# alex-petrenko/megaverse

Measured on NVIDIA H100. Metric: agent obs/sec (whole box), higher is better.
Workload: dtype f32

## Files before the change

### megaverse_b200/capi.py

```python
import ctypes as C
import os

import numpy as np

_PKG = os.path.dirname(os.path.abspath(__file__))
LIB_PATH = os.environ.get("MV_B200_LIB") or os.path.join(_PKG, "libmegaverse_b200.so")
_lib = None

MV_OK, MV_ERR_ARG, MV_ERR_CUDA, MV_ERR_CAPACITY, MV_ERR_STATE = 0, -1, -2, -3, -4
MV_END_NONE, MV_END_TIME, MV_END_SOLVED, MV_END_REQUESTED = 0, 1, 2, 3
MV_SEG_NONE, MV_SEG_STATIC, MV_SEG_TERRAIN, MV_SEG_OBJECT, MV_SEG_AGENT, MV_SEG_REWARD = 0, 1, 2, 3, 4, 5


class MegaverseError(RuntimeError):
    def __init__(self, code, msg):
        super().__init__("megaverse_b200 error %d: %s" % (code, msg))
        self.code = code


def lib():
    global _lib
    if _lib is None:
        if not os.path.exists(LIB_PATH):
            raise ImportError("%s is missing: run `python -m megaverse_b200._build` (needs nvcc)" % LIB_PATH)
# ... 382 lines not shown

    def static_cap(self):
        lib().mv_debug_static_cap.argtypes = [C.c_void_p]
        return int(lib().mv_debug_static_cap(self._h))

    def raster_config(self):
        out = (C.c_int32 * 4)()
        lib().mv_debug_raster_config.argtypes = [C.c_void_p, C.c_void_p]
        self._ck(lib().mv_debug_raster_config(self._h, out))
        return {"grid": out[0], "ctas_per_sm": out[1], "smem": out[2], "bands": out[3]}

    def raster_stats(self, enable=True, read=True):
        out = (C.c_ulonglong * 16)()
        lib().mv_debug_raster_stats.argtypes = [C.c_void_p, C.c_void_p, C.c_int]
        self._ck(lib().mv_debug_raster_stats(self._h, out if read else None, 1 if enable else 0))
        names = ["work_items", "instances", "visible_instances", "items", "clipped_items", "triangles", "batches", "sub_passes", "cyc_head", "cyc_tma_wait", "cyc_instance", "cyc_item", "cyc_tile", "cyc_total"]
        return {n: int(out[i]) for i, n in enumerate(names)}

    def states_create(self, rows):
        sid = C.c_int()
        self._ck(lib().mv_states_create(self._h, int(rows), C.byref(sid)))
        return sid.value

    def states_save(self, store, envs, rows):
        e, r = np.ascontiguousarray(envs, dtype=np.int32), np.ascontiguousarray(rows, dtype=np.int32)
        assert e.size == r.size
        self._ck(lib().mv_states_save(self._h, int(store), e.ctypes.data, r.ctypes.data, e.size))

    def states_load(self, store, rows, envs):
        r, e = np.ascontiguousarray(rows, dtype=np.int32), np.ascontiguousarray(envs, dtype=np.int32)
        assert e.size == r.size
# ... 130 lines not shown
```

### megaverse_b200/csrc/engine.cu

```cuda
#include <cuda_runtime.h>

#include <algorithm>
#include <atomic>
#include <cctype>
#include <cmath>
#include <condition_variable>
#include <cstddef>
#include <cstdio>
#include <cstring>
#include <deque>
#include <functional>
#include <map>
#include <memory>
#include <mutex>
#include <optional>
#include <queue>
#include <string>
#include <thread>
#include <vector>

#include "../../include/megaverse_b200.h"
#include "hostmath.hpp"
#include "level_set.h"
#include "levelgen.hpp"
// ... 111 lines not shown
        std::vector<MvLevel> level;
        std::vector<std::vector<MvBox>> statics;
        std::vector<std::vector<float>> staticRot;
        std::vector<std::vector<MvDeco>> deco;
        std::vector<std::vector<uint32_t>> solid;
    };
    std::vector<HostRow> host;
    void free() { for (auto &s : slabs) s.free(); for (auto &s : stateSlabs) s.free(); }
};

}

static void fillConsts(MvConsts &k, int W, int H);
static_assert(MV_STATE_OBJECT_ROWS == MV_MAX_OBJECTS && MV_STATE_REWARD_ROWS == MV_MAX_REWARD, "state tensor rows");

static mvr::ViewParams frameParams(int W, int H, int bands, int bandRows, unsigned long long *spill, int triCap, const MvConsts &k) {
    mvr::ViewParams vp = {};
    vp.W = W; vp.H = H; vp.bands = bands; vp.bandRows = bandRows; vp.spill = spill; vp.spillStride = W * bandRows; vp.triCap = triCap;
    vp.p00 = k.p00; vp.p11 = k.p11; vp.p22 = k.p22; vp.p32 = k.p32;
    return vp;
}

constexpr int kMaxRasterWidth = 768;

static int hiresBandRows(int w) { return std::max(1, 96 / (w / 32)) * 4; }
static bool hiresSizeOk(int w, int hgt) { return w >= 32 && hgt >= 4 && w % 32 == 0 && hgt % 4 == 0 && w <= kMaxRasterWidth && hgt <= 4096; }
template <typename B> static cudaError_t ensureCapacity(B &b, size_t count) {
    if (b.p && b.n >= count) return cudaSuccess;
    b.free();
    return b.alloc(count);
}

using ViewKernel = void (*)(mvr::ViewParams);
// ... 15 lines not shown
}

struct mv_engine {
    std::string error;
    void setError(const std::string &e) { error = e; }

    int W = 0, H = 0, E = 0, A = 0, N = 0, threads = 1, device = 0;
    std::vector<std::string> envScenarioName;
    std::vector<int> envScenario;
    std::vector<std::vector<std::pair<std::string, float>>> shaping;
    std::vector<mv::LevelGenerator> gens;
    std::mt19937 master{std::random_device{}()};
    std::unique_ptr<WorkerPool> pool;

    int gridCells = 0, gridWords = 0;
    int triCap = 368;
    std::atomic<int> maxObjSeen{0};
    bool wantDepth = false, obsToHost = true, didReset = false, fastShading = true;
    bool wantSeg = false;
    bool hostStepPending = false;
    bool skipUnfitLevels = false;
    std::atomic<int> levelsSkipped{0};
    int zeroCopyOpt = 1, hostSlicesOpt = 0;
    bool rasterToHost = false;
    bool deliverToHost = false;
    bool deviceObsFresh = false;
    bool hostObsFresh = false, ownDeviceObsFresh = false;
    bool ownDeviceBuffers() const { return obsOut == d_obs.p && (!wantDepth || depthOut == d_depth.p); }
    int sliceCount = 1;
    cudaStream_t copyStream = nullptr;
    std::vector<cudaEvent_t> sliceEv;
// ... 35 lines not shown
    DevBuf<int32_t> d_actions;
    DevBuf<float> d_rtable;
    DevBuf<float> d_rewards;
    DevBuf<uint8_t> d_dones;
    DevBuf<uint8_t> d_doneReasons;
    DevBuf<float> d_trueObj;
    DevBuf<uint8_t> d_obs;
    DevBuf<float> d_depth;
    DevBuf<uint16_t> d_seg;
    uint8_t *obsOut = nullptr;
    float *depthOut = nullptr;
    DevBuf<int32_t> d_faults;
    DevBuf<uint32_t> d_workCounter;
    uint32_t counterBase = 0;
    DevBuf<unsigned long long> d_spill;
    DevBuf<unsigned long long> d_rasterStats;
    DevBuf<uint32_t> d_viewCost;
    size_t costItems() const { return size_t(N) * size_t(H / 4); }
    int rasterGridCap = 0;
    int rasterSched = 1;
    int rasterGrid = 0, rasterCtasPerSM = 0, rasterBands = 1, bandRows = 0;
    size_t rasterSmem = 0;
    struct Hires {
        int W = 0, H = 0;
        DevBuf<uint8_t> d_obs; PinBuf<uint8_t> h_obs;
        DevBuf<unsigned long long> spill;
        void free() { d_obs.free(); h_obs.free(); spill.free(); W = H = 0; }
    } hires;
    struct Cameras {
        DevBuf<int32_t> d_env; DevBuf<float> d_views;
// ... 359 lines not shown
            if (timed) MV_CUDA(cudaEventRecord(evRays, stream));
            if (const int rc = castRays(false, sp.active)) return rc;
            if (final) { if (const int rc = castRays(true, nullptr)) return rc; }
        }
        if (const int rc = endTimes(dep ? Timed::Union : Timed::Split, timed, final, nRays > 0)) return rc;
        return (nRays && !async) ? downloadRays(stream) : MV_OK;
    }
    int endTimes(Timed kind, bool timed = true, bool hadFinal = false, bool hadRays = false) {
        if (timed) MV_CUDA(cudaEventRecord(ev[2], stream));
        timedAs = kind;
        lastHadFinal = timed && hadFinal;
        lastHadRays = timed && hadRays;
        return MV_OK;
    }
    int launchFinal(bool toHost) {
        mvr::ViewParams vp = frameParams(W, H, rasterBands, bandRows, d_spill.p, triCap, consts);
        vp.instances = d_termInst.p; vp.instCounts = d_termCounts.p; vp.views = d_termViews.p;
        vp.obs = toHost ? h_finalObs.p : d_finalObs.p; vp.depth = wantDepth ? (toHost ? h_finalDepth.p : d_finalDepth.p) : nullptr;
        vp.viewBase = 0; vp.N = N;
        vp.envMask = d_dones.p;
        finalOnDevice = !toHost;
        return launchView(vp, false, mvr::Items::Ended);
    }
    int rasterGridFor(const mvr::ViewParams &vp) const {
        const int full = vp.camEnv ? cameraGrid : (vp.envMask ? maskedGrid : rasterGrid);
        return std::min(rasterGridCap > 0 ? std::min(full, rasterGridCap) : full, vp.N * vp.bands);
    }
    int launchView(mvr::ViewParams &vp, bool dependent, mvr::Items items = mvr::Items::All) {
        const int grid = rasterGridFor(vp);
        vp.A = A; vp.instStride = instCap;
        vp.workCounter = d_workCounter.p; vp.counterBase = counterBase;
// ... 2 lines not shown
        cfg.gridDim = dim3(unsigned(grid)); cfg.blockDim = dim3(mvr::kThreads); cfg.dynamicSmemBytes = rasterSmem; cfg.stream = stream;
        cudaLaunchAttribute attr[1];
        attr[0].id = cudaLaunchAttributeProgrammaticStreamSerialization;
        attr[0].val.programmaticStreamSerializationAllowed = 1;
        cfg.attrs = attr; cfg.numAttrs = dependent ? 1 : 0;
        MV_CUDA(cudaLaunchKernelEx(&cfg, viewKernelOf(items, vp.seg != nullptr, fastShading), vp));
        launches += 1;
        return MV_OK;
    }
    cudaError_t resetViewOrder() {
        std::vector<uint32_t> init(costItems() + size_t(E) + 1, 0u);
        for (int e = 0; e < E; ++e) init[costItems() + size_t(e)] = uint32_t(e);
        return cudaMemcpy(d_viewCost.p, init.data(), sizeof(uint32_t) * init.size(), cudaMemcpyHostToDevice);
    }
    int launchRaster(bool dep, const uint8_t *active) {
        mvr::ViewParams vp = frameParams(W, H, rasterBands, bandRows, d_spill.p, triCap, consts);
        vp.instances = d_inst.p; vp.instCounts = d_instCounts.p; vp.views = d_views.p;
        vp.obs = rasterToHost ? h_obs.p : obsOut; vp.depth = wantDepth ? (rasterToHost ? h_depth.p : depthOut) : nullptr;
        vp.seg = wantSeg ? (rasterToHost ? h_seg.p : d_seg.p) : nullptr;
        vp.stats = d_rasterStats.p;
        vp.ready = dep ? d_ready.p : nullptr; vp.readyStamp = dep ? readyStamp : 0;
        const bool fresh = rasterToHost ? hostObsFresh : (ownDeviceObsFresh && ownDeviceBuffers());
        const uint8_t *mask = fresh ? active : nullptr;
        const mvr::Items items = mask ? mvr::Items::Active : mvr::Items::All;
        vp.envMask = mask;
        deviceObsFresh = !rasterToHost;
        ownDeviceObsFresh = !rasterToHost && ownDeviceBuffers();
        hostObsFresh = deliverToHost;
        if (sliceCount <= 1) {
            vp.viewBase = 0; vp.N = N;
            if (rasterSched == 2 || (rasterSched == 1 && N * rasterBands > rasterGridFor(vp))) {
// ... 56 lines not shown
        vp.instances = d_inst.p; vp.instCounts = d_instCounts.p; vp.views = d_views.p;
        vp.obs = hires.d_obs.p;
        vp.viewBase = 0; vp.N = N;
        rc = launchView(vp, false);
        if (rc) return rc;
        MV_CUDA(cudaMemcpyAsync(hires.h_obs.p, hires.d_obs.p, size_t(N) * w * hgt * 4, cudaMemcpyDeviceToHost, stream));
        MV_CUDA(cudaStreamSynchronize(stream));
        return MV_OK;
    }
    int bandedFrame(int w, int hgt, int grid, DevBuf<unsigned long long> &spill, mvr::ViewParams &vp) {
        const int rowsPerBand = hiresBandRows(w);
        const int bands = (hgt + rowsPerBand - 1) / rowsPerBand;
        if (ensureCapacity(spill, size_t(grid) * w * rowsPerBand) != cudaSuccess) { setError("raster spill slab allocation failed"); return MV_ERR_CUDA; }
        MvConsts k;
        fillConsts(k, w, hgt);
        vp = frameParams(w, hgt, bands, rowsPerBand, spill.p, triCap, k);
        return MV_OK;
    }
    int launchCameras(const int32_t *dEnv, const float *dViews, int n, int w, int hgt, uint8_t *obs, float *depth, uint16_t *seg) {
        if (ensureCapacity(cams.d_range, 1) != cudaSuccess) { setError("camera counter allocation failed"); return MV_ERR_CUDA; }
        MV_CUDA(cudaMemsetAsync(cams.d_range.p, 0, sizeof(uint32_t), stream));
        if (n == 0) return MV_OK;
        mvr::ViewParams vp;
        const int rc = bandedFrame(w, hgt, cameraGrid, cams.spill, vp);
        if (rc) return rc;
        vp.instances = d_inst.p; vp.instCounts = d_instCounts.p; vp.views = dViews;
        vp.obs = obs; vp.depth = depth; vp.seg = seg;
        vp.viewBase = 0; vp.N = n;
        vp.camEnv = dEnv; vp.numEnvs = E; vp.rangeCount = cams.d_range.p;
        return launchView(vp, false, mvr::Items::Cameras);
    }
// ... 84 lines not shown
            maskedPerSM = v ? std::min(maskedPerSM, perSM) : perSM;
        }
        maskedGrid = numSMs * std::max(1, std::min(maskedPerSM, rasterCtasPerSM));
        int cameraPerSM = 0;
        for (int v = 0; v < 4; ++v) {
            const void *fn = reinterpret_cast<const void *>(viewKernelOf(mvr::Items::Cameras, v >= 2, v & 1));
            MV_CUDA(cudaFuncSetAttribute(fn, cudaFuncAttributeMaxDynamicSharedMemorySize, maxOptin));
            int perSM = 0;
            MV_CUDA(cudaOccupancyMaxActiveBlocksPerMultiprocessor(&perSM, fn, mvr::kThreads, rasterSmem));
            cameraPerSM = v ? std::min(cameraPerSM, perSM) : perSM;
        }
        cameraGrid = numSMs * std::max(1, std::min(cameraPerSM, rasterCtasPerSM));
        bandRows = ((H / 4 + rasterBands - 1) / rasterBands) * 4;
        d_spill.free();
        if (d_spill.alloc(size_t(rasterGrid) * W * bandRows) != cudaSuccess) { setError("raster spill slab allocation failed"); return MV_ERR_CUDA; }
        hires.free();
        return MV_OK;
    }

    void afterFlip(const uint8_t *flipped) {
        const int D = levelSlots;
        for (int e = 0; e < E; ++e) {
            if (!flipped || flipped[e]) {
                if (levelSet) { hostEpisode[size_t(e)] += 1; continue; }
                hostSlot[size_t(e)] = (hostSlot[size_t(e)] + 1) % D;
                hostEpisode[size_t(e)] += 1;
                scheduleGen(e, (hostSlot[size_t(e)] + D - 1) % D, hostEpisode[size_t(e)] + D - 1);
            }
        }
    }
// ... 347 lines not shown
        const int rc = quiesce();
        if (rc) return rc;
        MV_CUDA(cudaMemcpyAsync(&d_agents.p[size_t(env) * A + agent], w16, sizeof(float) * 16, cudaMemcpyHostToDevice, stream));
        MV_CUDA(cudaStreamSynchronize(stream));
        return MV_OK;
    }

    void freeAll() {
        if (pool) { pool->waitAll(); pool.reset(); }
        for (auto &st : stores) if (st) st->free();
        stores.clear();
        d_bankBase.free(); d_levelIds.free(); d_nextLevels.free(); h_levelIds.free(); h_nextLevels.free();
        h_pairs.free(); d_pairs.free(); h_envList.free(); d_envList.free(); h_active.free(); d_active.free();
        d_levels.free(); d_statics.free(); d_staticRot.free(); h_statics.free(); h_staticRot.free(); d_solid.free(); d_objGrid.free(); d_envs.free(); d_agents.free(); d_objects.free(); d_inst.free(); d_instCounts.free();
        d_views.free(); d_actions.free(); d_rtable.free(); d_rewards.free(); d_dones.free(); d_trueObj.free(); d_obs.free(); d_depth.free(); d_seg.free(); d_faults.free();
        hires.free(); cams.free(); d_deco.free(); h_deco.free(); d_prof.free(); d_ready.free(); d_workCounter.free(); d_spill.free(); d_rasterStats.free(); d_viewCost.free();
        h_levels.free(); h_solid.free(); h_actions.free(); h_rtable.free(); h_rewards.free(); h_dones.free(); h_trueObj.free(); h_obs.free(); h_depth.free(); h_seg.free();
        h_faults.free(); h_faultWord.free();
        d_doneReasons.free(); h_doneReasons.free();
        d_termInst.free(); d_termCounts.free(); d_termViews.free(); d_finalObs.free(); d_finalDepth.free(); h_finalObs.free(); h_finalDepth.free();
        d_state.free(); h_state.free();
        if (evState) { cudaEventDestroy(evState); evState = nullptr; }
        d_rayDirs.free(); d_rayDist.free(); d_rayTag.free(); h_rayDist.free(); h_rayTag.free();
        if (evRays) { cudaEventDestroy(evRays); evRays = nullptr; }
        for (auto &e : ev) if (e) { cudaEventDestroy(e); e = nullptr; }
        if (evFinal) { cudaEventDestroy(evFinal); evFinal = nullptr; }
        for (auto &p : ring) { if (p.ev) { cudaEventDestroy(p.ev); p.ev = nullptr; } p.rewards.free(); p.trueObj.free(); p.dones.free(); p.reasons.free(); p.levelIds.free(); }
        for (auto &e2 : sliceEv) if (e2) cudaEventDestroy(e2);
        sliceEv.clear();
        if (copyStream) { cudaStreamDestroy(copyStream); copyStream = nullptr; }
        if (stream) { cudaStreamDestroy(stream); stream = nullptr; }
// ... 1138 lines not shown
    int32_t cnt[8] = {0, n, 0, 0, 0, 0, 0, 0};
    for (int i = 0, last = 0; i < n; ++i) {
        MvInstance &d = inst[size_t(i)];
        d.mesh = int(inst18[i * 18]); d.color = int(inst18[i * 18 + 1]);
        std::memcpy(d.model, inst18 + i * 18 + 2, 64);
        d.pad[0] = i + 1; d.pad[1] = 0;
        if (d.mesh < last || d.mesh > 4 || d.color < 0 || d.color >= 22) return MV_ERR_ARG;
        last = d.mesh;
        cnt[d.mesh == 0 ? 0 : 1 + d.mesh] += 1;
    }
    MvConsts k;
    fillConsts(k, w, h);
    if (uploadPalette(&tmp) != MV_OK) return MV_ERR_CUDA;
    const ViewKernel fn = viewKernelOf(mvr::Items::All, wantSeg, fast);
    MvInstance *dInst = nullptr; int32_t *dCnt = nullptr; float *dView = nullptr, *dDepth = nullptr; uint8_t *dObs = nullptr; uint16_t *dSeg = nullptr;
    uint32_t *dCtr = nullptr; unsigned long long *dSpill = nullptr, *dStats = nullptr;
    const size_t px = size_t(w) * size_t(h);
    bool ok = cudaMalloc(&dInst, sizeof(MvInstance) * inst.size()) == cudaSuccess && cudaMalloc(&dCnt, 32) == cudaSuccess &&
              cudaMalloc(&dView, 64) == cudaSuccess && cudaMalloc(&dObs, px * 4) == cudaSuccess && cudaMalloc(&dDepth, px * 4) == cudaSuccess &&
              cudaMalloc(&dSeg, px * 2) == cudaSuccess && cudaMalloc(&dStats, 16 * sizeof(unsigned long long)) == cudaSuccess &&
              cudaMalloc(&dCtr, 16) == cudaSuccess && cudaMalloc(&dSpill, sizeof(unsigned long long) * size_t(bands) * size_t(w) * bandRows) == cudaSuccess &&
              cudaFuncSetAttribute(reinterpret_cast<const void *>(fn), cudaFuncAttributeMaxDynamicSharedMemorySize, maxOptin) == cudaSuccess;
    if (ok) {
        cudaMemcpy(dInst, inst.data(), sizeof(MvInstance) * inst.size(), cudaMemcpyHostToDevice);
        cudaMemcpy(dCnt, cnt, 32, cudaMemcpyHostToDevice);
        cudaMemcpy(dView, view16, 64, cudaMemcpyHostToDevice);
        cudaMemset(dCtr, 0, 16);
        cudaMemset(dStats, 0, 16 * sizeof(unsigned long long));
        mvr::ViewParams vp = frameParams(w, h, bands, bandRows, dSpill, triCap, k);
        vp.instances = dInst; vp.instCounts = dCnt; vp.views = dView; vp.instStride = int(inst.size()); vp.obs = dObs; vp.depth = depth ? dDepth : nullptr;
        vp.seg = wantSeg ? dSeg : nullptr; vp.stats = stats ? dStats : nullptr;
        vp.workCounter = dCtr; vp.viewBase = 0; vp.N = 1; vp.A = 1;
        fn<<<bands, mvr::kThreads, smem>>>(vp);
        ok = cudaDeviceSynchronize() == cudaSuccess;
        if (ok) {
            cudaMemcpy(rgba, dObs, px * 4, cudaMemcpyDeviceToHost);
            if (depth) cudaMemcpy(depth, dDepth, px * 4, cudaMemcpyDeviceToHost);
            if (wantSeg) cudaMemcpy(seg, dSeg, px * 2, cudaMemcpyDeviceToHost);
            if (stats) cudaMemcpy(stats, dStats, 16 * sizeof(unsigned long long), cudaMemcpyDeviceToHost);
        }
    }
    cudaFree(dCtr); cudaFree(dSpill); cudaFree(dInst); cudaFree(dCnt); cudaFree(dView); cudaFree(dObs); cudaFree(dDepth); cudaFree(dSeg); cudaFree(dStats);
    return ok ? MV_OK : MV_ERR_CUDA;
}

int mv_debug_render_instances(const float *view16, const float *inst18, int n, int w, int h, uint8_t *rgba, float *depth) {
    if (w < 32 || h < 4 || w % 32 || h % 4 || (w / 32) * (h / 4) > 128) return MV_ERR_ARG;
    const int opts[4] = {0, 0, 96, (h / 4) % 2 == 0 ? 2 : 1};
    return mv_debug_render_instances_ex(view16, inst18, n, w, h, opts, rgba, depth, nullptr, nullptr);
}

int mv_debug_cast_rays(const float *views16, const float *inst18, const int32_t *tags, const int32_t *counts, int E, int A, int stride,
                       const float *dirs3, int R, float max_dist, const uint8_t *env_mask, float *dist, uint16_t *tag) {
    if (!views16 || !inst18 || !tags || !counts || !dirs3 || !dist || !tag) return MV_ERR_ARG;
    if (E < 1 || E > 65536 || A < 1 || A > MV_MAX_AGENTS || R < 1 || R > MV_MAX_RAYS || stride < 1 || stride > 65536) return MV_ERR_ARG;
    if (size_t(E) * size_t(stride) > (size_t(1) << 22) || !std::isfinite(max_dist) || !(max_dist > 0.0f)) return MV_ERR_ARG;
    std::vector<MvInstance> inst(size_t(E) * size_t(stride));
// ... 70 lines not shown
```

### megaverse_b200/csrc/raster_view.cuh

```cuda
#pragma once
#include "dev_math.cuh"
#include "mesh_tables.inc"
#include "mv_types.h"

namespace mvr {
using namespace dm;

struct __align__(16) TriCover {
    long long C[3];
    int32_t A[3], B[3];
    float z[3];
    float invArea;
    uint32_t key;
    int32_t flags;
    uint32_t bx, by;
};
struct __align__(16) TriShade {
    float rw[3];
    float p[9];
    float n[9];
    float diffuse[3];
};
static_assert(sizeof(TriCover) == 80 && sizeof(TriShade) == 96, "triangle record layout");

// ... 44 lines not shown
    unsigned long long *stats;
    uint32_t *viewCost;
    uint32_t *order;
    uint32_t *exitCounter;
    unsigned long long *spill;
    int spillStride;
    int viewBase, N;
    int A, W, H;
    int bands, bandRows;
    int triCap;
    float p00, p11, p22, p32;
    const uint8_t *envMask;
    const int32_t *camEnv;
    uint32_t *rangeCount;
    int numEnvs;
};

struct SmemLayout { uint32_t stage, cover, shade, xf, off, frag, small, meshV, meshI, clip, slow, sched, misc, total; };
struct ViewMisc {
    float view[16];
    int32_t counts[8];
    int32_t nTris;
    int32_t nValid;
    int32_t tileCtr;
    uint32_t claim;
    int32_t prefetched;
    int32_t lastCta;
    int32_t wsum[kWarps];
    int32_t nSlow[2];
    uint32_t stat[8];
    alignas(8) unsigned long long bar[2];
    unsigned long long itemStart;
};
__host__ __device__ inline SmemLayout smemLayout(int triCap) {
    SmemLayout L;
    uint32_t o = 0;
    L.stage = o; o += 2u * kInstChunk * uint32_t(sizeof(MvInstance));
    L.cover = o; o += uint32_t(triCap) * uint32_t(sizeof(TriCover));
    L.shade = o; o += uint32_t(triCap) * uint32_t(sizeof(TriShade));
    L.xf = o; o += uint32_t(kXfWords) * kInstChunk * 4u;
    L.off = o; o += (kInstChunk + 4u) * 4u;
    L.frag = o; o += uint32_t(kWarps) * 128u * 8u;
    L.meshV = o; o += uint32_t(kMeshVerts) * 6u * 4u;
    L.meshI = o; o += (uint32_t(kMeshIdx) + 15u) & ~15u;
    L.clip = L.frag;
    L.small = o; o += uint32_t(kWarps) * kSmallList * 2u;
    L.slow = o; o += 2u * kThreads * 2u;
    L.sched = o; o += 256u * 4u;
    L.misc = o; o += (uint32_t(sizeof(ViewMisc)) + 15u) & ~15u;
    L.total = o;
    return L;
}

__device__ __forceinline__ uint32_t smemAddrOf(const void *p) { return uint32_t(__cvta_generic_to_shared(p)); }
__device__ __forceinline__ void mbarInit(unsigned long long *bar, int count) {
    asm volatile("mbarrier.init.shared::cta.b64 [%0], %1;" ::"r"(smemAddrOf(bar)), "r"(count));
    asm volatile("fence.mbarrier_init.release.cluster;" ::: "memory");
}
__device__ __forceinline__ void mbarExpectTx(unsigned long long *bar, uint32_t bytes) {
    asm volatile("mbarrier.arrive.expect_tx.shared::cta.b64 _, [%0], %1;" ::"r"(smemAddrOf(bar)), "r"(bytes) : "memory");
}
__device__ __forceinline__ void bulkG2S(void *dst, const void *src, uint32_t bytes, unsigned long long *bar) {
    asm volatile("cp.async.bulk.shared::cluster.global.mbarrier::complete_tx::bytes [%0], [%1], %2, [%3];" ::"r"(smemAddrOf(dst)), "l"(src), "r"(bytes),
                 "r"(smemAddrOf(bar))
                 : "memory");
}
__device__ __forceinline__ void mbarWait(unsigned long long *bar, uint32_t parity) {
// ... 110 lines not shown
    s.rw[0] = a.rw; s.rw[1] = b.rw; s.rw[2] = c.rw;
    s.p[0] = va.px; s.p[1] = va.py; s.p[2] = va.pz; s.p[3] = vb.px; s.p[4] = vb.py; s.p[5] = vb.pz; s.p[6] = vc.px; s.p[7] = vc.py; s.p[8] = vc.pz;
    s.n[0] = va.nx; s.n[1] = va.ny; s.n[2] = va.nz; s.n[3] = vb.nx; s.n[4] = vb.ny; s.n[5] = vb.nz; s.n[6] = vc.nx; s.n[7] = vc.ny; s.n[8] = vc.nz;
    const bool flat = va.nx == vb.nx && va.ny == vb.ny && va.nz == vb.nz && va.nx == vc.nx && va.ny == vc.ny && va.nz == vc.nz;
    if (FAST && flat) {
        const float inv = rsqrtf(va.nx * va.nx + va.ny * va.ny + va.nz * va.nz);
        s.n[0] = va.nx * inv; s.n[1] = va.ny * inv; s.n[2] = va.nz * inv;
    }
    cv.invArea = 1.0f / float(-tb.area2);
    cv.key = key;
    cv.flags = tl | (worst < (1ll << 30) ? 8 : 0) | (flat ? 16 : 0) | (colorTag & int(0xffff0000u));
    cv.bx = tb.bx;
    cv.by = tb.by;
    s.diffuse[0] = c_palette[color][0]; s.diffuse[1] = c_palette[color][1]; s.diffuse[2] = c_palette[color][2];
    cx.cover[slot] = cv;
    cx.shade[slot] = s;
}

__device__ __forceinline__ void vertPosition(ClipVert &cv, const float mv[12], const float *vp, float p00, float p11, float p22, float p32) {
    { float acc = 0.0f; acc += mv[0] * vp[0]; acc += mv[3] * vp[1]; acc += mv[6] * vp[2]; acc += mv[9] * 1.0f; cv.px = acc; }
    { float acc = 0.0f; acc += mv[1] * vp[0]; acc += mv[4] * vp[1]; acc += mv[7] * vp[2]; acc += mv[10] * 1.0f; cv.py = acc; }
    { float acc = 0.0f; acc += mv[2] * vp[0]; acc += mv[5] * vp[1]; acc += mv[8] * vp[2]; acc += mv[11] * 1.0f; cv.pz = acc; }
    cv.cx = cv.px * p00;
    cv.cy = cv.py * p11;
    cv.cz = cv.pz * p22 + p32;
    cv.cw = -cv.pz;
}
__device__ __forceinline__ void vertNormal(ClipVert &cv, const float nm[9], const float *vp) {
    cv.nx = nm[0] * vp[3] + nm[3] * vp[4] + nm[6] * vp[5];
    cv.ny = nm[1] * vp[3] + nm[4] * vp[4] + nm[7] * vp[5];
    cv.nz = nm[2] * vp[3] + nm[5] * vp[4] + nm[8] * vp[5];
// ... 105 lines not shown
    return uint32_t(floorf(c * 255.0f + 0.5f));
}

template <bool FAST> __device__ __forceinline__ float invLen3(float x, float y, float z) {
    if (FAST) return rsqrtf(__fmaf_rn(z, z, __fmaf_rn(y, y, x * x)));
    return 1.0f / sqrtf((x * x + y * y) + z * z);
}
template <bool FAST> __device__ __forceinline__ float dot3(float ax, float ay, float az, float bx, float by, float bz) {
    if (FAST) return __fmaf_rn(az, bz, __fmaf_rn(ay, by, ax * bx));
    return (ax * bx + ay * by) + az * bz;
}

struct ShadeRec { float4 a0, a1, a2, a3, a4, a5; };
__device__ __forceinline__ ShadeRec loadShade(const TriShade *tp) {
    const float4 *q = reinterpret_cast<const float4 *>(tp);
    ShadeRec r;
    r.a0 = q[0]; r.a1 = q[1]; r.a2 = q[2]; r.a3 = q[3]; r.a4 = q[4]; r.a5 = q[5];
    return r;
}
template <bool FAST> __device__ __forceinline__ uint32_t shadePixel(const ShadeRec &rec, float l0, float l1, float l2, bool flat, float &wOut) {
    const float4 a0 = rec.a0, a1 = rec.a1, a2 = rec.a2, a3 = rec.a3, a4 = rec.a4, a5 = rec.a5;
    const float rw0 = a0.x, rw1 = a0.y, rw2 = a0.z;
    const float k0 = l0 * rw0, k1 = l1 * rw1, k2 = l2 * rw2;
    const float s = (k0 + k1) + k2;
    const float r = 1.0f / s;
    wOut = r;
    float Pc[3], nn0, nn1, nn2;
    if (FAST) {
        const float p[9] = {a0.w, a1.x, a1.y, a1.z, a1.w, a2.x, a2.y, a2.z, a2.w};
        const float q0 = k0 * r, q1 = k1 * r, q2 = k2 * r;
// ... 90 lines not shown
}
__device__ __forceinline__ unsigned long long packFrag(float z, uint32_t key, int idx) {
    const uint32_t b = __float_as_uint(z);
    const uint32_t asc = b ^ ((b >> 31) ? 0xffffffffu : 0x80000000u);
    return ((unsigned long long)(~asc) << 32) | (unsigned long long)((key << kIdxBits) | uint32_t(idx));
}

#ifdef MV_TILE_FORCEINLINE
#define MV_TILE_INLINE __forceinline__
#else
#define MV_TILE_INLINE __noinline__
#endif
extern __shared__ __align__(128) unsigned char g_viewSmem[];

template <bool FAST, bool SEG>
__device__ MV_TILE_INLINE void tilePass(const ViewParams &P, int count, unsigned long long *spill, int view, int rowLo, int bandTiles, int batch, bool final) {
    const SmemLayout L = smemLayout(P.triCap);
    const TriCover *cover = reinterpret_cast<const TriCover *>(g_viewSmem + L.cover);
    const TriShade *shade = reinterpret_cast<const TriShade *>(g_viewSmem + L.shade);
    unsigned long long *frag = reinterpret_cast<unsigned long long *>(g_viewSmem + L.frag) + (threadIdx.x >> 5) * 128;
    uint16_t *smallList = reinterpret_cast<uint16_t *>(g_viewSmem + L.small) + (threadIdx.x >> 5) * kSmallList;
    int32_t *tileCtr = &reinterpret_cast<ViewMisc *>(g_viewSmem + L.misc)->tileCtr;
    const int lane = threadIdx.x & 31;
    const int tilesX = P.W >> 5;
    for (;;) {
        int tile = 0;
        if (lane == 0) tile = atomicAdd(tileCtr, 1);
        tile = __shfl_sync(0xffffffffu, tile, 0);
        if (tile >= bandTiles) break;
        const int tk = tile / tilesX, ty = tk;
        const int tx0 = (tile - tk * tilesX) * 32, ty0 = rowLo + ty * 4;
        const int px = tx0 + (lane & 7) * 4, py = ty0 + (lane >> 3);
        const int sx32 = px * 256 + 128, sy32 = py * 256 + 128;
        unsigned long long best[4] = {0ull, 0ull, 0ull, 0ull};
// ... 208 lines not shown
    }
    return c;
}

#ifdef MV_VIEW_MAXNREG
#define MV_VIEW_BOUNDS __maxnreg__(MV_VIEW_MAXNREG)
#else
#define MV_VIEW_BOUNDS __launch_bounds__(kThreads, MV_VIEW_MIN_CTAS)
#endif
template <bool FAST, Items ITEMS = Items::All, bool SEG = false> __global__ void MV_VIEW_BOUNDS viewKernel(const __grid_constant__ ViewParams P) {
    constexpr bool CAM = ITEMS == Items::Cameras;
    unsigned char *smem = g_viewSmem;
    const SmemLayout L = smemLayout(P.triCap);
    MvInstance *stage = reinterpret_cast<MvInstance *>(smem + L.stage);
    TriCover *cover = reinterpret_cast<TriCover *>(smem + L.cover);
    TriShade *shade = reinterpret_cast<TriShade *>(smem + L.shade);
    float *xf = reinterpret_cast<float *>(smem + L.xf);
    int32_t *off = reinterpret_cast<int32_t *>(smem + L.off);
    float *meshV = reinterpret_cast<float *>(smem + L.meshV);
    uint8_t *meshI = smem + L.meshI;
    uint16_t *slowAll = reinterpret_cast<uint16_t *>(smem + L.slow);
    ClipVert *clipScratch = reinterpret_cast<ClipVert *>(smem + L.clip + (threadIdx.x >> 5) * 1024u);
    static_assert(4 * kClipVerts * sizeof(ClipVert) <= 1024, "a warp's clip polygons share its fragment buffer");
    ViewMisc &M = *reinterpret_cast<ViewMisc *>(smem + L.misc);
    const int tid = threadIdx.x, lane = tid & 31, warp = tid >> 5;

    for (int i = tid; i < kMeshVerts * 6; i += kThreads) {
        const int v = i / 6, c = i - v * 6;
        float val;
        if (v < kVCapsule) val = c_boxVerts[v][c];
        else if (v < kVSphere) val = c_capsuleVerts[v - kVCapsule][c];
// ... 40 lines not shown
                const uint32_t *flag = P.ready + env;
                uint32_t v;
                while (true) {
                    asm volatile("ld.acquire.gpu.global.u32 %0, [%1];" : "=r"(v) : "l"(flag) : "memory");
                    if (v == P.readyStamp) break;
                    __nanosleep(200);
                }
                asm volatile("fence.proxy.async;" ::: "memory");
            }
            M.itemStart = (unsigned long long)clock64();
            M.nTris = 0;
            M.nValid = 0x7fffffff;
            M.tileCtr = 0;
            M.nSlow[0] = 0; M.nSlow[1] = 0;
            for (int q = 0; q < 8; ++q) M.stat[q] = 0;
        }
        __syncthreads();
        if (!prefetched) {
            if (tid < 16) M.view[tid] = __ldcg(P.views + size_t(view) * 16 + tid);
            else if (tid < 24) M.counts[tid - 16] = live ? __ldcg(P.instCounts + env * 8 + (tid - 16)) : 0;
            __syncthreads();
        }
        const int nInst = M.counts[1];
        const int nChunks = (nInst + kInstChunk - 1) / kInstChunk;
        if (tid == 0 && nChunks > 0 && !prefetched) {
            const uint32_t bytes = uint32_t(min(nInst, kInstChunk)) * uint32_t(sizeof(MvInstance));
            mbarExpectTx(&M.bar[0], bytes);
            bulkG2S(stage, inst, bytes, &M.bar[0]);
        }
        M4 viewM;
// ... 217 lines not shown
                            int base = 0;
                            if (lane == 0) base = reserveTris(cx, __popc(vm));
                            base = __shfl_sync(0xffffffffu, base, 0);
                            if (base < 0) done = false;
                            else if (vis) writeTri<FAST>(cx, base + __popc(vm & ((1u << lane) - 1u)), pp[0], pp[k], pp[k + 1], sa, sb, sc, tb, color, keyBase + uint32_t(t));
                        }
                        if (done) { if (lane == 0) slowList[sidx] = uint16_t(e | 0x8000); }
                        else slowFull = true;
                        if (CAM && done && band == 0 && P.rangeCount) {
                            const unsigned wm = __ballot_sync(0xffffffffu, wide);
                            if (lane == 0 && wm) atomicAdd(P.rangeCount, uint32_t(__popc(wm)));
                        }
                        __syncwarp();
                    }
                    if (!__syncthreads_or((pending || slowFull) ? 1 : 0)) break;
                    tilePass<FAST, SEG>(P, min(M.nTris, M.nValid), spill, view, rowLo, bandTiles, batch, false);
                    if (P.stats && tid == 0) M.stat[5] += uint32_t(min(M.nTris, M.nValid));
                    ++batch;
                    again = true;
                    __syncthreads();
                    if (tid == 0) { M.nTris = 0; M.nValid = 0x7fffffff; M.tileCtr = 0; }
                    __syncthreads();
                }
            }
            __syncthreads();
            if (P.stats) tcItem += clock64() - tw2;
        }
        const long long tc2 = P.stats ? clock64() : 0;
        if (tid == 0) {
            const uint32_t nc = claimWork<ITEMS>(P, total);
            int pre = 0;
            if (nc < total) {
                const int nview = P.viewBase + int(nc / uint32_t(bands)), nenv = CAM ? P.camEnv[nview] : nview / P.A;
                const bool nlive = !CAM || (nenv >= 0 && nenv < P.numEnvs);
                bool ready = true;
// ... 13 lines not shown
#pragma unroll
                    for (int q = 0; q < 16; ++q) M.view[q] = vm[q];
#pragma unroll
                    for (int q = 0; q < 8; ++q) M.counts[q] = cn[q];
                    if (cn[1] > 0) {
                        const uint32_t bytes = uint32_t(min(cn[1], kInstChunk)) * uint32_t(sizeof(MvInstance));
                        mbarExpectTx(&M.bar[0], bytes);
                        bulkG2S(stage, P.instances + size_t(nenv) * size_t(P.instStride), bytes, &M.bar[0]);
                    }
                    pre = 1;
                }
            }
            M.claim = nc; M.prefetched = pre;
        }
        if (live) {
            tilePass<FAST, SEG>(P, min(M.nTris, M.nValid), spill, view, rowLo, bandTiles, batch, true);
        } else {
            const size_t px0 = (size_t(view) * P.H + size_t(rowLo)) * P.W;
            for (int q = tid; q < ((rowHi - rowLo + 1) * P.W) >> 2; q += kThreads) {
                const size_t p = px0 + size_t(q) * 4;
                *reinterpret_cast<uint4 *>(P.obs + p * 4) = make_uint4(0u, 0u, 0u, 0u);
                if (P.depth) *reinterpret_cast<float4 *>(P.depth + p) = make_float4(0.0f, 0.0f, 0.0f, 0.0f);
                if (SEG) *reinterpret_cast<uint2 *>(P.seg + p) = make_uint2(0u, 0u);
            }
        }
        __syncthreads();
        if (P.viewCost && tid == 0) P.viewCost[claim] = uint32_t(min((unsigned long long)clock64() - M.itemStart, 0xffffffffull * 16ull) >> 4);
        if (P.stats && tid < 8) {
            unsigned long long v = M.stat[tid];
            if (tid == 0) v = 1;
            if (tid == 5) v += (unsigned long long)min(M.nTris, M.nValid);
            if (tid == 6) v = (unsigned long long)(batch + 1);
            atomicAdd(P.stats + tid, v);
            if (tid == 0) {
                const long long tc3 = clock64();
                atomicAdd(P.stats + 8, (unsigned long long)(tc1 - tc0)); atomicAdd(P.stats + 9, (unsigned long long)tcWait);
                atomicAdd(P.stats + 10, (unsigned long long)tcInst); atomicAdd(P.stats + 11, (unsigned long long)tcItem);
                atomicAdd(P.stats + 12, (unsigned long long)(tc3 - tc2)); atomicAdd(P.stats + 13, (unsigned long long)(tc3 - tc0));
            }
        }
    }
    if (P.viewCost) {
        if (tid == 0) {
            __threadfence();
            M.lastCta = atomicAdd(P.exitCounter, 1u) == gridDim.x - 1u ? 1 : 0;
        }
        __syncthreads();
        if (M.lastCta) {
            __threadfence();
            uint32_t *bins = reinterpret_cast<uint32_t *>(smem + L.sched);
            const int E = P.N / P.A;
            uint32_t *costS = reinterpret_cast<uint32_t *>(smem + L.cover);
            const int capS = int((L.xf - L.cover) / 4u);
            const bool inSmem = E <= capS;
            if (inSmem) {
                for (int e = tid; e < E; e += kThreads) costS[e] = 0u;
                __syncthreads();
                const uint32_t perEnv = uint32_t(P.A) * uint32_t(P.bands);
                const int items = int(total);
                for (int v0 = tid; v0 < items; v0 += 4 * kThreads) {
                    uint32_t c[4];
#pragma unroll
                    for (int q = 0; q < 4; ++q) { const int v = v0 + q * kThreads; c[q] = v < items ? __ldcg(P.viewCost + v) : 0u; }
#pragma unroll
                    for (int q = 0; q < 4; ++q) { const int v = v0 + q * kThreads; if (v < items) atomicAdd(&costS[uint32_t(v) / perEnv], c[q]); }
                }
                __syncthreads();
            }
// ... 47 lines not shown
```

Baseline: 2.902 million.

## Move per-triangle shading records from shared memory to a per-CTA global slab

Triangle shading records (TriShade) now live in a per-CTA global-memory slab instead of shared memory, so the shared layout holds only cover records. The default triangle capacity is derived at compile time from the shared-memory budget and minimum CTAs per SM, so a CTA can hold more triangles per batch and may need fewer mid-band tile passes. The cost is that shading reads in the tile pass go through L1/L2 rather than shared memory. A stats counter for mid-batch tile-pass cycles is also added.

```diff
diff --git a/megaverse_b200/capi.py b/megaverse_b200/capi.py
--- a/megaverse_b200/capi.py
+++ b/megaverse_b200/capi.py
@@ -420,7 +420,7 @@
         out = (C.c_ulonglong * 16)()
         lib().mv_debug_raster_stats.argtypes = [C.c_void_p, C.c_void_p, C.c_int]
         self._ck(lib().mv_debug_raster_stats(self._h, out if read else None, 1 if enable else 0))
-        names = ["work_items", "instances", "visible_instances", "items", "clipped_items", "triangles", "batches", "sub_passes", "cyc_head", "cyc_tma_wait", "cyc_instance", "cyc_item", "cyc_tile", "cyc_total"]
+        names = ["work_items", "instances", "visible_instances", "items", "clipped_items", "triangles", "batches", "sub_passes", "cyc_head", "cyc_tma_wait", "cyc_instance", "cyc_item", "cyc_tile", "cyc_total", "cyc_mid_tile"]
         return {n: int(out[i]) for i, n in enumerate(names)}
 
     def states_create(self, rows):
diff --git a/megaverse_b200/csrc/engine.cu b/megaverse_b200/csrc/engine.cu
--- a/megaverse_b200/csrc/engine.cu
+++ b/megaverse_b200/csrc/engine.cu
@@ -149,9 +149,11 @@
 static void fillConsts(MvConsts &k, int W, int H);
 static_assert(MV_STATE_OBJECT_ROWS == MV_MAX_OBJECTS && MV_STATE_REWARD_ROWS == MV_MAX_REWARD, "state tensor rows");
 
-static mvr::ViewParams frameParams(int W, int H, int bands, int bandRows, unsigned long long *spill, int triCap, const MvConsts &k) {
+static mvr::ViewParams frameParams(int W, int H, int bands, int bandRows, unsigned long long *spill, int triCap, mvr::TriShade *shade,
+                                   const MvConsts &k) {
     mvr::ViewParams vp = {};
     vp.W = W; vp.H = H; vp.bands = bands; vp.bandRows = bandRows; vp.spill = spill; vp.spillStride = W * bandRows; vp.triCap = triCap;
+    vp.shade = shade; vp.shadeStride = triCap;
     vp.p00 = k.p00; vp.p11 = k.p11; vp.p22 = k.p22; vp.p32 = k.p32;
     return vp;
 }
@@ -197,7 +199,7 @@
     std::unique_ptr<WorkerPool> pool;
 
     int gridCells = 0, gridWords = 0;
-    int triCap = 368;
+    int triCap = mvr::kDefaultTriCap;
     std::atomic<int> maxObjSeen{0};
     bool wantDepth = false, obsToHost = true, didReset = false, fastShading = true;
     bool wantSeg = false;
@@ -263,6 +265,7 @@
     DevBuf<uint32_t> d_workCounter;
     uint32_t counterBase = 0;
     DevBuf<unsigned long long> d_spill;
+    DevBuf<mvr::TriShade> d_shade;
     DevBuf<unsigned long long> d_rasterStats;
     DevBuf<uint32_t> d_viewCost;
     size_t costItems() const { return size_t(N) * size_t(H / 4); }
@@ -652,7 +655,7 @@
         return MV_OK;
     }
     int launchFinal(bool toHost) {
-        mvr::ViewParams vp = frameParams(W, H, rasterBands, bandRows, d_spill.p, triCap, consts);
+        mvr::ViewParams vp = frameParams(W, H, rasterBands, bandRows, d_spill.p, triCap, d_shade.p, consts);
         vp.instances = d_termInst.p; vp.instCounts = d_termCounts.p; vp.views = d_termViews.p;
         vp.obs = toHost ? h_finalObs.p : d_finalObs.p; vp.depth = wantDepth ? (toHost ? h_finalDepth.p : d_finalDepth.p) : nullptr;
         vp.viewBase = 0; vp.N = N;
@@ -685,7 +688,7 @@
         return cudaMemcpy(d_viewCost.p, init.data(), sizeof(uint32_t) * init.size(), cudaMemcpyHostToDevice);
     }
     int launchRaster(bool dep, const uint8_t *active) {
-        mvr::ViewParams vp = frameParams(W, H, rasterBands, bandRows, d_spill.p, triCap, consts);
+        mvr::ViewParams vp = frameParams(W, H, rasterBands, bandRows, d_spill.p, triCap, d_shade.p, consts);
         vp.instances = d_inst.p; vp.instCounts = d_instCounts.p; vp.views = d_views.p;
         vp.obs = rasterToHost ? h_obs.p : obsOut; vp.depth = wantDepth ? (rasterToHost ? h_depth.p : depthOut) : nullptr;
         vp.seg = wantSeg ? (rasterToHost ? h_seg.p : d_seg.p) : nullptr;
@@ -772,7 +775,7 @@
         if (ensureCapacity(spill, size_t(grid) * w * rowsPerBand) != cudaSuccess) { setError("raster spill slab allocation failed"); return MV_ERR_CUDA; }
         MvConsts k;
         fillConsts(k, w, hgt);
-        vp = frameParams(w, hgt, bands, rowsPerBand, spill.p, triCap, k);
+        vp = frameParams(w, hgt, bands, rowsPerBand, spill.p, triCap, d_shade.p, k);
         return MV_OK;
     }
     int launchCameras(const int32_t *dEnv, const float *dViews, int n, int w, int hgt, uint8_t *obs, float *depth, uint16_t *seg) {
@@ -887,6 +890,8 @@
         bandRows = ((H / 4 + rasterBands - 1) / rasterBands) * 4;
         d_spill.free();
         if (d_spill.alloc(size_t(rasterGrid) * W * bandRows) != cudaSuccess) { setError("raster spill slab allocation failed"); return MV_ERR_CUDA; }
+        d_shade.free();
+        if (d_shade.alloc(size_t(rasterGrid) * size_t(triCap)) != cudaSuccess) { setError("raster shading slab allocation failed"); return MV_ERR_CUDA; }
         hires.free();
         return MV_OK;
     }
@@ -1264,7 +1269,7 @@
         h_pairs.free(); d_pairs.free(); h_envList.free(); d_envList.free(); h_active.free(); d_active.free();
         d_levels.free(); d_statics.free(); d_staticRot.free(); h_statics.free(); h_staticRot.free(); d_solid.free(); d_objGrid.free(); d_envs.free(); d_agents.free(); d_objects.free(); d_inst.free(); d_instCounts.free();
         d_views.free(); d_actions.free(); d_rtable.free(); d_rewards.free(); d_dones.free(); d_trueObj.free(); d_obs.free(); d_depth.free(); d_seg.free(); d_faults.free();
-        hires.free(); cams.free(); d_deco.free(); h_deco.free(); d_prof.free(); d_ready.free(); d_workCounter.free(); d_spill.free(); d_rasterStats.free(); d_viewCost.free();
+        hires.free(); cams.free(); d_deco.free(); h_deco.free(); d_prof.free(); d_ready.free(); d_workCounter.free(); d_spill.free(); d_shade.free(); d_rasterStats.free(); d_viewCost.free();
         h_levels.free(); h_solid.free(); h_actions.free(); h_rtable.free(); h_rewards.free(); h_dones.free(); h_trueObj.free(); h_obs.free(); h_depth.free(); h_seg.free();
         h_faults.free(); h_faultWord.free();
         d_doneReasons.free(); h_doneReasons.free();
@@ -2433,12 +2438,13 @@
     if (uploadPalette(&tmp) != MV_OK) return MV_ERR_CUDA;
     const ViewKernel fn = viewKernelOf(mvr::Items::All, wantSeg, fast);
     MvInstance *dInst = nullptr; int32_t *dCnt = nullptr; float *dView = nullptr, *dDepth = nullptr; uint8_t *dObs = nullptr; uint16_t *dSeg = nullptr;
-    uint32_t *dCtr = nullptr; unsigned long long *dSpill = nullptr, *dStats = nullptr;
+    uint32_t *dCtr = nullptr; unsigned long long *dSpill = nullptr, *dStats = nullptr; mvr::TriShade *dShade = nullptr;
     const size_t px = size_t(w) * size_t(h);
     bool ok = cudaMalloc(&dInst, sizeof(MvInstance) * inst.size()) == cudaSuccess && cudaMalloc(&dCnt, 32) == cudaSuccess &&
               cudaMalloc(&dView, 64) == cudaSuccess && cudaMalloc(&dObs, px * 4) == cudaSuccess && cudaMalloc(&dDepth, px * 4) == cudaSuccess &&
               cudaMalloc(&dSeg, px * 2) == cudaSuccess && cudaMalloc(&dStats, 16 * sizeof(unsigned long long)) == cudaSuccess &&
               cudaMalloc(&dCtr, 16) == cudaSuccess && cudaMalloc(&dSpill, sizeof(unsigned long long) * size_t(bands) * size_t(w) * bandRows) == cudaSuccess &&
+              cudaMalloc(&dShade, sizeof(mvr::TriShade) * size_t(bands) * size_t(triCap)) == cudaSuccess &&
               cudaFuncSetAttribute(reinterpret_cast<const void *>(fn), cudaFuncAttributeMaxDynamicSharedMemorySize, maxOptin) == cudaSuccess;
     if (ok) {
         cudaMemcpy(dInst, inst.data(), sizeof(MvInstance) * inst.size(), cudaMemcpyHostToDevice);
@@ -2446,7 +2452,7 @@
         cudaMemcpy(dView, view16, 64, cudaMemcpyHostToDevice);
         cudaMemset(dCtr, 0, 16);
         cudaMemset(dStats, 0, 16 * sizeof(unsigned long long));
-        mvr::ViewParams vp = frameParams(w, h, bands, bandRows, dSpill, triCap, k);
+        mvr::ViewParams vp = frameParams(w, h, bands, bandRows, dSpill, triCap, dShade, k);
         vp.instances = dInst; vp.instCounts = dCnt; vp.views = dView; vp.instStride = int(inst.size()); vp.obs = dObs; vp.depth = depth ? dDepth : nullptr;
         vp.seg = wantSeg ? dSeg : nullptr; vp.stats = stats ? dStats : nullptr;
         vp.workCounter = dCtr; vp.viewBase = 0; vp.N = 1; vp.A = 1;
@@ -2459,7 +2465,7 @@
             if (stats) cudaMemcpy(stats, dStats, 16 * sizeof(unsigned long long), cudaMemcpyDeviceToHost);
         }
     }
-    cudaFree(dCtr); cudaFree(dSpill); cudaFree(dInst); cudaFree(dCnt); cudaFree(dView); cudaFree(dObs); cudaFree(dDepth); cudaFree(dSeg); cudaFree(dStats);
+    cudaFree(dCtr); cudaFree(dSpill); cudaFree(dShade); cudaFree(dInst); cudaFree(dCnt); cudaFree(dView); cudaFree(dObs); cudaFree(dDepth); cudaFree(dSeg); cudaFree(dStats);
     return ok ? MV_OK : MV_ERR_CUDA;
 }
 
diff --git a/megaverse_b200/csrc/raster_view.cuh b/megaverse_b200/csrc/raster_view.cuh
--- a/megaverse_b200/csrc/raster_view.cuh
+++ b/megaverse_b200/csrc/raster_view.cuh
@@ -82,9 +82,11 @@
     const int32_t *camEnv;
     uint32_t *rangeCount;
     int numEnvs;
+    TriShade *shade;
+    int shadeStride;
 };
 
-struct SmemLayout { uint32_t stage, cover, shade, xf, off, frag, small, meshV, meshI, clip, slow, sched, misc, total; };
+struct SmemLayout { uint32_t stage, cover, xf, off, frag, small, meshV, meshI, clip, slow, sched, misc, total; };
 struct ViewMisc {
     float view[16];
     int32_t counts[8];
@@ -99,13 +101,13 @@
     uint32_t stat[8];
     alignas(8) unsigned long long bar[2];
     unsigned long long itemStart;
+    unsigned long long midStart, midCycles;
 };
-__host__ __device__ inline SmemLayout smemLayout(int triCap) {
-    SmemLayout L;
+__host__ __device__ constexpr SmemLayout smemLayout(int triCap) {
+    SmemLayout L{};
     uint32_t o = 0;
     L.stage = o; o += 2u * kInstChunk * uint32_t(sizeof(MvInstance));
     L.cover = o; o += uint32_t(triCap) * uint32_t(sizeof(TriCover));
-    L.shade = o; o += uint32_t(triCap) * uint32_t(sizeof(TriShade));
     L.xf = o; o += uint32_t(kXfWords) * kInstChunk * 4u;
     L.off = o; o += (kInstChunk + 4u) * 4u;
     L.frag = o; o += uint32_t(kWarps) * 128u * 8u;
@@ -119,6 +121,10 @@
     L.total = o;
     return L;
 }
+constexpr uint32_t kSmemPerSM = 228u * 1024u, kSmemReservedPerCta = 1024u;
+constexpr int kDefaultTriCap =
+    int((kSmemPerSM / MV_VIEW_MIN_CTAS - kSmemReservedPerCta - smemLayout(0).total) / uint32_t(sizeof(TriCover)));
+static_assert(kDefaultTriCap >= 32 && kDefaultTriCap <= kMaxTriCap, "default triangle-list capacity within the tri_cap range");
 
 __device__ __forceinline__ uint32_t smemAddrOf(const void *p) { return uint32_t(__cvta_generic_to_shared(p)); }
 __device__ __forceinline__ void mbarInit(unsigned long long *bar, int count) {
@@ -259,7 +265,11 @@
     cv.by = tb.by;
     s.diffuse[0] = c_palette[color][0]; s.diffuse[1] = c_palette[color][1]; s.diffuse[2] = c_palette[color][2];
     cx.cover[slot] = cv;
-    cx.shade[slot] = s;
+    const float4 *q = reinterpret_cast<const float4 *>(&s);
+    float4 *d = reinterpret_cast<float4 *>(cx.shade + slot);
+    __builtin_assume(__isGlobal(d));
+#pragma unroll
+    for (int i = 0; i < 6; ++i) d[i] = q[i];
 }
 
 __device__ __forceinline__ void vertPosition(ClipVert &cv, const float mv[12], const float *vp, float p00, float p11, float p22, float p32) {
@@ -395,6 +405,7 @@
 struct ShadeRec { float4 a0, a1, a2, a3, a4, a5; };
 __device__ __forceinline__ ShadeRec loadShade(const TriShade *tp) {
     const float4 *q = reinterpret_cast<const float4 *>(tp);
+    __builtin_assume(__isGlobal(q));
     ShadeRec r;
     r.a0 = q[0]; r.a1 = q[1]; r.a2 = q[2]; r.a3 = q[3]; r.a4 = q[4]; r.a5 = q[5];
     return r;
@@ -515,10 +526,9 @@
 extern __shared__ __align__(128) unsigned char g_viewSmem[];
 
 template <bool FAST, bool SEG>
-__device__ MV_TILE_INLINE void tilePass(const ViewParams &P, int count, unsigned long long *spill, int view, int rowLo, int bandTiles, int batch, bool final) {
+__device__ MV_TILE_INLINE void tilePass(const ViewParams &P, int count, unsigned long long *spill, const TriShade *shade, int view, int rowLo, int bandTiles, int batch, bool final) {
     const SmemLayout L = smemLayout(P.triCap);
     const TriCover *cover = reinterpret_cast<const TriCover *>(g_viewSmem + L.cover);
-    const TriShade *shade = reinterpret_cast<const TriShade *>(g_viewSmem + L.shade);
     unsigned long long *frag = reinterpret_cast<unsigned long long *>(g_viewSmem + L.frag) + (threadIdx.x >> 5) * 128;
     uint16_t *smallList = reinterpret_cast<uint16_t *>(g_viewSmem + L.small) + (threadIdx.x >> 5) * kSmallList;
     int32_t *tileCtr = &reinterpret_cast<ViewMisc *>(g_viewSmem + L.misc)->tileCtr;
@@ -757,7 +767,7 @@
     const SmemLayout L = smemLayout(P.triCap);
     MvInstance *stage = reinterpret_cast<MvInstance *>(smem + L.stage);
     TriCover *cover = reinterpret_cast<TriCover *>(smem + L.cover);
-    TriShade *shade = reinterpret_cast<TriShade *>(smem + L.shade);
+    TriShade *shade = P.shade + size_t(blockIdx.x) * size_t(P.shadeStride);
     float *xf = reinterpret_cast<float *>(smem + L.xf);
     int32_t *off = reinterpret_cast<int32_t *>(smem + L.off);
     float *meshV = reinterpret_cast<float *>(smem + L.meshV);
@@ -828,6 +838,7 @@
             M.tileCtr = 0;
             M.nSlow[0] = 0; M.nSlow[1] = 0;
             for (int q = 0; q < 8; ++q) M.stat[q] = 0;
+            M.midCycles = 0;
         }
         __syncthreads();
         if (!prefetched) {
@@ -1075,11 +1086,13 @@
                         __syncwarp();
                     }
                     if (!__syncthreads_or((pending || slowFull) ? 1 : 0)) break;
-                    tilePass<FAST, SEG>(P, min(M.nTris, M.nValid), spill, view, rowLo, bandTiles, batch, false);
+                    if (P.stats && tid == 0) M.midStart = (unsigned long long)clock64();
+                    tilePass<FAST, SEG>(P, min(M.nTris, M.nValid), spill, shade, view, rowLo, bandTiles, batch, false);
                     if (P.stats && tid == 0) M.stat[5] += uint32_t(min(M.nTris, M.nValid));
                     ++batch;
                     again = true;
                     __syncthreads();
+                    if (P.stats && tid == 0) M.midCycles += (unsigned long long)clock64() - M.midStart;
                     if (tid == 0) { M.nTris = 0; M.nValid = 0x7fffffff; M.tileCtr = 0; }
                     __syncthreads();
                 }
@@ -1123,7 +1136,7 @@
             M.claim = nc; M.prefetched = pre;
         }
         if (live) {
-            tilePass<FAST, SEG>(P, min(M.nTris, M.nValid), spill, view, rowLo, bandTiles, batch, true);
+            tilePass<FAST, SEG>(P, min(M.nTris, M.nValid), spill, shade, view, rowLo, bandTiles, batch, true);
         } else {
             const size_t px0 = (size_t(view) * P.H + size_t(rowLo)) * P.W;
             for (int q = tid; q < ((rowHi - rowLo + 1) * P.W) >> 2; q += kThreads) {
@@ -1144,8 +1157,9 @@
             if (tid == 0) {
                 const long long tc3 = clock64();
                 atomicAdd(P.stats + 8, (unsigned long long)(tc1 - tc0)); atomicAdd(P.stats + 9, (unsigned long long)tcWait);
-                atomicAdd(P.stats + 10, (unsigned long long)tcInst); atomicAdd(P.stats + 11, (unsigned long long)tcItem);
+                atomicAdd(P.stats + 10, (unsigned long long)tcInst); atomicAdd(P.stats + 11, (unsigned long long)tcItem - M.midCycles);
                 atomicAdd(P.stats + 12, (unsigned long long)(tc3 - tc2)); atomicAdd(P.stats + 13, (unsigned long long)(tc3 - tc0));
+                atomicAdd(P.stats + 14, M.midCycles);
             }
         }
     }
@@ -1159,8 +1173,8 @@
             __threadfence();
             uint32_t *bins = reinterpret_cast<uint32_t *>(smem + L.sched);
             const int E = P.N / P.A;
-            uint32_t *costS = reinterpret_cast<uint32_t *>(smem + L.cover);
-            const int capS = int((L.xf - L.cover) / 4u);
+            uint32_t *costS = reinterpret_cast<uint32_t *>(smem + L.stage);
+            const int capS = int((L.xf - L.stage) / 4u);
             const bool inSmem = E <= capS;
             if (inSmem) {
                 for (int e = tid; e < E; e += kThreads) costS[e] = 0u;
```

New measurement: 3.006 million, median of 6. +3.6%, better.
